# taaha-khan/2023-CompaCT-Image-Compression

Measured on AMD Instinct MI355X. Metric: MPixels/s encode+decode, 12-bit 512x512 CT batch, bytes-exact, higher is better.
Workload: dtype u16

## Files before the change

2023-compact-image-compression_amd/csrc/api.cpp:

```cpp
#include <dlfcn.h>
#include <unistd.h>
#include <zlib.h>

#include <atomic>
#include <chrono>
#include <condition_variable>
#include <functional>
#include <cstdarg>
#include <cstdio>
#include <cstdlib>
#include <cstring>
#include <map>
#include <mutex>
#include <string>
#include <thread>
#include <vector>

#include "../../include/compact_hip.h"
#include "cct_internal.h"
#include "host.h"
#include "handoff.h"

namespace cct {
bool gilbert_table(int width, int height, int32_t *out);
// ... 619 lines not shown
		return CCT_OK;
	}
	if (tb && tb->tiled) {
		bool tile_role_in_lds = true;
		(void)enc_tiles_lds_bytes(NB, &tile_role_in_lds);
		if (!tile_role_in_lds) { if ((rc = E.e_role.ensure(per))) return rc; a.ws_role = (uint8_t *)E.e_role.p; }
		else a.ws_role = nullptr;
		TileEncArgs ta{};
		ta.e = a;
		ta.tile_org = tb->d_org; ta.tile_orient = tb->d_orient; ta.patterns = tb->d_pat;
		ta.n_orient = tb->n_orient; ta.n_tiles = tb->n_tiles; ta.row_pitch = width;
		HIP_TRY(launch_encode_tiles(ta, n, st));
		g_ctx.last_path = 2;
		return CCT_OK;
	}
	const bool run_time = bs_run_time(bs, g_ctx.runtime_bs != 0);
	HIP_TRY(launch_encode(a, n, bs, g_ctx.wg_threads, st, run_time));
	g_ctx.last_path = run_time ? 4 : 0;
	return CCT_OK;
}

constexpr size_t DEFLATE_PASS_BYTES = (size_t)1 << 30;

int deflate_locked(EncSlot &E, const uint8_t *d_in, size_t in_stride, const uint32_t *d_in_sizes, int n, const uint8_t header13[13],
                   size_t out_stride, int level, int strategy, int mem_level = 8)
{
	if (in_stride % 256 != 0 || out_stride % 4 != 0) return fail(CCT_E_ARG, "deflate strides must be multiples of 256 / 4");
	DeflateArgs a{};
	if (!deflate_strategy_args(level, strategy, a))
		return fail(CCT_E_ARG, "zlib level %d with strategy %d is not on the device", level, strategy);
	if (!deflate_mem_level_args(mem_level, a)) return fail(CCT_E_ARG, "zlib memLevel %d: 8 and 9 are on the device", mem_level);
	const size_t EB = (size_t)n * in_stride;
	if (EB >= ((size_t)1 << 32)) return fail(CCT_E_ARG, "deflate batch of %zu bytes exceeds the 4 GiB sort limit; split the batch", EB);
	const DflShape shape = dfl_shape(n, in_stride, a.block_syms);
	int rc;
	void *base[DFL_REGIONS];
	for (int r = 0; r < DFL_REGIONS; r++) {
		if (dfl_region_needed(r, strategy) && (rc = E.z_ws[r].ensure(dfl_region_bytes(r, shape)))) return rc;
		base[r] = E.z_ws[r].p;
	}
	if ((rc = E.z_out.ensure((size_t)n * out_stride))) return rc;
	if ((rc = E.z_outsizes.ensure((size_t)n * 4))) return rc;
	const bool use_fork = g_ctx.deflate_fork != 0;
	if (use_fork && !E.stream_side) {
		const int crc = exclusive_section([&]() -> int { HIP_TRY(hipStreamCreateWithFlags(&E.stream_side, hipStreamNonBlocking)); return CCT_OK; });
		if (crc) return crc;
	}
	a.in = d_in; a.in_stride = in_stride; a.in_sizes = d_in_sizes;
	dfl_bind(a, base, shape);
	a.tree_waves = (uint32_t)g_ctx.tree_waves;
	a.pos_mask = (g_ctx.compact_recs && mem_level == 8 && in_stride < ((size_t)1 << 22)) ? (1u << 22) - 1u : 0xFFFFFFFFu;
	const DevBuf &mr = E.z_ws[DFL_R_MATCH];
	if (dfl_uses_chains(strategy)) {
		if (E.z_mr_cleared != mr.p || E.z_mr_cleared_cap != mr.cap || E.z_gen_passes >= 16000u) {
			HIP_TRY(hipMemsetAsync(mr.p, 0, mr.cap, E.stream));
			HIP_TRY(hipMemsetAsync(E.z_ws[DFL_R_GEN].p, 0, 256, E.stream));
			E.z_mr_cleared = mr.p; E.z_mr_cleared_cap = mr.cap; E.z_gen_passes = 0;
		}
		E.z_gen_passes++;
	}
	a.out = (uint8_t *)E.z_out.p; a.out_stride = out_stride; a.out_sizes = (uint32_t *)E.z_outsizes.p;
	memcpy(a.header13, header13, 13);
	if (g_ctx.use_graph) {
		std::vector<uint8_t> key(sizeof(DeflateArgs) + 2 * sizeof(int));
		memcpy(key.data(), &a, sizeof(DeflateArgs));
		memcpy(key.data() + sizeof(DeflateArgs), &n, sizeof(int));
		const int fork_key = use_fork ? 1 : 0;
		memcpy(key.data() + sizeof(DeflateArgs) + sizeof(int), &fork_key, sizeof(int));
		EncSlot::ZGraph *zg = nullptr;
		for (auto &g : E.z_graphs) if (g.key == key) zg = &g;
		if (!zg) {
			const int crc = exclusive_section([&]() -> int {
				if (E.z_graphs.size() >= 4) {
					size_t old = 0;
					for (size_t i = 1; i < E.z_graphs.size(); i++) if (E.z_graphs[i].last_use < E.z_graphs[old].last_use) old = i;
					if (E.z_graphs[old].exec) (void)hipGraphExecDestroy(E.z_graphs[old].exec);
					if (E.z_graphs[old].graph) (void)hipGraphDestroy(E.z_graphs[old].graph);
					E.z_graphs.erase(E.z_graphs.begin() + (long)old);
				}
				EncSlot::ZGraph g;
				HIP_TRY(hipStreamBeginCapture(E.stream, hipStreamCaptureModeThreadLocal));
				hipError_t le = launch_deflate(a, n, E.stream, use_fork ? E.stream_side : nullptr, E.ev_fork);
				hipError_t ce = hipStreamEndCapture(E.stream, &g.graph);
				if (le != hipSuccess) { if (g.graph) (void)hipGraphDestroy(g.graph); return fail(CCT_E_DEVICE, "DEFLATE capture: %s", hipGetErrorString(le)); }
				HIP_TRY(ce);
				const hipError_t ie = hipGraphInstantiate(&g.exec, g.graph, nullptr, nullptr, 0);
				if (ie != hipSuccess) { (void)hipGraphDestroy(g.graph); return fail(CCT_E_DEVICE, "hipGraphInstantiate failed: %s", hipGetErrorString(ie)); }
				g.key = key;
				E.z_graphs.push_back(std::move(g));
				return CCT_OK;
			});
			if (crc) return crc;
			zg = &E.z_graphs.back();
		}
		zg->last_use = ++E.z_clock;
		HIP_TRY(hipGraphLaunch(zg->exec, E.stream));
		return CCT_OK;
	}
	HIP_TRY(launch_deflate(a, n, E.stream, use_fork ? E.stream_side : nullptr, E.ev_fork));
	return CCT_OK;
}

int decode_payload_locked(DecSlot &D, const uint8_t *d_payload, size_t stride, const uint32_t *d_sizes, int n, int width,
                          int height, int bs, int fractal, uint16_t *d_images, uint32_t *d_status, hipStream_t st)
{
	const int N = width * height, NB = N / bs;
	if (stride % 16 != 0) return fail(CCT_E_ARG, "payload stride must be a multiple of 16");
// ... 1416 lines not shown
```

2023-compact-image-compression_amd/csrc/deflate_kernels.hip:

```cpp
#include <hip/hip_runtime.h>
#include <cstring>
#include <algorithm>

#include "cct_internal.h"
#include "wave_device.h"
#include "../../include/compact_hip.h"

namespace cct {
namespace {

constexpr int MIN_MATCH = 3, MAX_MATCH = 258, WSIZE = 32768;
constexpr int MIN_LOOKAHEAD = MAX_MATCH + MIN_MATCH + 1;
constexpr int MAX_DIST = WSIZE - MIN_LOOKAHEAD;
constexpr int TOO_FAR = 4096;
constexpr int BLOCK_SYMS = 16383;
constexpr int BLOCK_SYMS_ML9 = 32767;
constexpr int L_CODES = 286, D_CODES = 30, BL_CODES = 19, HEAP_SIZE = 2 * L_CODES + 1;
constexpr int END_BLOCK = 256, MAX_BITS = 15, MAX_BL_BITS = 7;
constexpr uint32_t Z_FILTERED = 1, Z_HUFFMAN_ONLY = 2, Z_RLE = 3, Z_FIXED = 4;
__host__ __device__ __forceinline__ bool short_pass(uint32_t strategy) { return strategy == Z_HUFFMAN_ONLY || strategy == Z_RLE; }

__constant__ uint8_t c_extra_lbits[29] = {0,0,0,0,0,0,0,0,1,1,1,1,2,2,2,2,3,3,3,3,4,4,4,4,5,5,5,5,0};
__constant__ uint8_t c_extra_dbits[30] = {0,0,0,0,1,1,2,2,3,3,4,4,5,5,6,6,7,7,8,8,9,9,10,10,11,11,12,12,13,13};
__constant__ uint8_t c_extra_blbits[19] = {0,0,0,0,0,0,0,0,0,0,0,0,0,0,0,0,2,3,7};
__constant__ uint8_t c_bl_order[19] = {16,17,18,0,8,7,9,6,10,5,11,4,12,3,13,2,14,1,15};
__constant__ uint8_t c_length_code[256];
__constant__ uint16_t c_base_length[29];
__constant__ uint8_t c_dist_code[512];
__constant__ uint16_t c_base_dist[30];
__constant__ uint16_t c_static_lcode[288];
__constant__ uint8_t c_static_llen[288];
__constant__ uint16_t c_static_dcode[30];

template <int HB>
__device__ __forceinline__ uint32_t hash3(uint32_t b0, uint32_t b1, uint32_t b2)
{
	constexpr int SH = (HB + 2) / 3;
	return ((b0 << (2 * SH)) ^ (b1 << SH) ^ b2) & ((1u << HB) - 1u);
}

__device__ __forceinline__ int d_code(uint32_t dist) { return dist < 256 ? c_dist_code[dist] : c_dist_code[256 + (dist >> 7)]; }

struct MatchRec { uint16_t len_full, len_quarter, dist_full, dist_quarter; };
constexpr uint32_t GEN_MAX = 16383;
__device__ __forceinline__ uint2 pack_match(uint32_t len_full, uint32_t len_quarter, uint32_t dist_full, uint32_t dist_quarter, uint32_t gen)
{
	return make_uint2((len_full | ((gen & 127u) << 9)) | ((len_quarter | ((gen >> 7) << 9)) << 16), dist_full | (dist_quarter << 16));
}
__device__ __forceinline__ MatchRec checked_match(MatchRec r, uint32_t gen, uint32_t rw, uint32_t p, uint32_t L)
{
	const uint32_t tag = (uint32_t)(r.len_full >> 9) | ((uint32_t)(r.len_quarter >> 9) << 7);
	const uint32_t lookahead = L - min(p, L);
	const uint32_t max_len = lookahead < (uint32_t)MAX_MATCH ? lookahead : (uint32_t)MAX_MATCH;
	const bool maximal = (rw >> 15) && (rw & 0x7FFFu) >= max_len && p + 2 < L;
	MatchRec o;
	const bool ok = tag == gen;
	o.len_full = ok ? (uint16_t)(r.len_full & 511u) : (uint16_t)(maximal ? max_len : 0u);
	o.len_quarter = ok ? (uint16_t)(r.len_quarter & 511u) : (uint16_t)(maximal ? max_len : 0u);
	o.dist_full = ok ? r.dist_full : (uint16_t)(maximal ? 1u : 0u);
	o.dist_quarter = ok ? r.dist_quarter : (uint16_t)(maximal ? 1u : 0u);
	return o;
}

template <bool FIRST, int HB>
__global__ void __launch_bounds__(1024) dfl_sort_pass_kernel(DeflateArgs a)
{
	constexpr int BITS = FIRST ? 8 : HB - 8, NB = 1 << BITS;
	constexpr uint32_t HMASK = (1u << HB) - 1u;
	__shared__ uint32_t offs[256];
	__shared__ uint32_t wcnt[16][NB];
	const int s = blockIdx.x;
	const uint32_t L = a.in_sizes[s];
	const uint8_t *in = a.in + (size_t)s * a.in_stride;
	const size_t base = (size_t)s * a.in_stride;
	const uint32_t npos = L >= MIN_MATCH ? L - 2 : 0;
	const uint64_t *rec_src = a.rec_in + base;
	uint64_t *rec_dst = (FIRST ? a.rec_in : a.rec_out) + base;
	const int tid = threadIdx.x, lane = tid & 63, wave = tid >> 6;
	const uint64_t lt_mask = (1ull << lane) - 1ull;
	if (tid < 256) offs[tid] = 0;
	__syncthreads();
	if (tid < NB) offs[tid] = a.sort_hist[(size_t)s * SORT_HIST + (FIRST ? 0 : 256) + tid];
	__syncthreads();
	if (wave == 0) {
		uint32_t v[4], sum = 0;
#pragma unroll
		for (int k = 0; k < 4; k++) { v[k] = offs[lane * 4 + k]; sum += v[k]; }
		uint32_t run = wave_incl_scan(sum) - sum;
#pragma unroll
		for (int k = 0; k < 4; k++) { offs[lane * 4 + k] = run; run += v[k]; }
	}
	__syncthreads();
#ifndef CCT_SORT_E
#define CCT_SORT_E 4
#endif
	constexpr int E = CCT_SORT_E;
	constexpr int ND = E / 4;
	const uint32_t last = npos ? npos - 1 : 0;
	static_assert(E % 4 == 0 && ND + 1 <= E, "pass A: whole dwords per lane, kept in ra[0 .. ND]");
#ifdef CCT_SORT_PROBE
	const bool compact = false;
#else
	const bool compact = HB == 15 && a.pos_mask != 0xFFFFFFFFu;
#endif
	const uint32_t dmax = (uint32_t)a.in_stride - 4u;
	auto fetch = [&](uint32_t tile_base, uint32_t (&ra)[E], uint32_t (&rb)[E]) {
		if (FIRST) {
#pragma unroll
			for (int d = 0; d < ND; d++) ra[d] = *reinterpret_cast<const uint32_t *>(in + min(tile_base + 256u * d + 4u * (uint32_t)lane, dmax));
			ra[ND] = *reinterpret_cast<const uint32_t *>(in + min(tile_base + 256u * ND, dmax));
#pragma unroll
			for (int e = 0; e < E; e++) rb[e] = compact ? a.run_len[base + min(tile_base + (uint32_t)(e * 64 + lane), last)] : 0u;
		} else {
// ... 259 lines not shown
		if ((rw >> 15) && (int)run_r >= nice_eff) { best = best1 = (int)run_r; best_q = best_q1 = p - 1; }
		else kind = 2;
		return;
	}
	for (int64_t j = (int64_t)i - 1; j >= 0; j--) {
		const uint64_t rj = recs[j];
		if (rec_hash(rj, pos_mask) != h) break;
		if (count == LIGHT_STEPS) { kind = 1; break; }
		const uint32_t q = rec_pos(rj, pos_mask);
		const uint32_t dist = p - q;
		if (q == 0 || q == nil_q) break;
		if (count == 0 ? dist > (uint32_t)MAX_DIST : dist >= (uint32_t)MAX_DIST) break;
		const uint8_t *mp = in + q;
		{
			int len = 0;
			if (wide) {
				if (best < 8 || mp[best] == sp[best]) {
					uint64_t cw;
					__builtin_memcpy(&cw, mp, 8);
					const uint64_t d = cw ^ ow;
					len = d ? (__ffsll((long long)d) - 1) >> 3 : common_prefix(mp, sp, 8, max_len);
				}
			} else if (mp[best] == sp[best]) len = common_prefix(mp, sp, 0, max_len);
			if (len > best) {
				best = len; best_q = q;
				if (count < quarter) { best1 = len; best_q1 = q; }
			}
		}
		count++;
		if (best >= nice_eff) break;
	}
}

#ifndef DFL_MATCH_Q
#define DFL_MATCH_Q 256
#endif
#ifndef DFL_MATCH_GRID
#define DFL_MATCH_GRID 32
#endif
constexpr uint32_t MATCH_Q = DFL_MATCH_Q;
static_assert(MATCH_Q >= 128 && (MATCH_Q & 63) == 0, "a turn appends up to 64 entries to a list");

template <bool CMP, bool QL>
__global__ void __launch_bounds__(256) dfl_match_kernel(DeflateArgs a, int n)
{
	__shared__ uint32_t queue[4][2][MATCH_Q];
	int s; uint32_t part, nparts;
	if (!xcd_slice(n, s, part, nparts)) return;
	const uint32_t L = a.in_sizes[s], gen = *a.gen;
	const uint8_t *in = a.in + (size_t)s * a.in_stride;
	const size_t base = (size_t)s * a.in_stride;
	const uint32_t npos = L >= MIN_MATCH ? L - 2 : 0;
	const uint64_t *recs = a.rec_out + base;
	uint2 *mr = reinterpret_cast<uint2 *>(a.mr) + base;
	uint32_t *heavy = a.heavy_list + base;
	const uint16_t *rl = a.run_len + base;
	const int lane = threadIdx.x & 63;
	const uint64_t lt_mask = (1ull << lane) - 1ull;
	const int quarter = QL ? (int)(a.max_chain >> 2) : LIGHT_STEPS + 1;
	const uint32_t stride = nparts * 256u;
	uint32_t i0 = part * 256u;
	if (i0 >= npos) return;
	uint32_t *qh = queue[threadIdx.x >> 6][0], *qr = queue[threadIdx.x >> 6][1];
	uint32_t nh = 0, nr = 0;
	auto flush = [&](const uint32_t *q, uint32_t cnt, uint32_t *counter, bool down) {
		uint32_t b = 0;
		if (lane == 0) b = atomicAdd(counter, cnt);
		b = (uint32_t)__builtin_amdgcn_readfirstlane((int)b);
		__builtin_amdgcn_wave_barrier();
		for (uint32_t k = (uint32_t)lane; k < cnt; k += 64u) {
			if (down) *(dfl_deep_top(heavy, a.in_stride) - (b + k)) = q[k];
			else heavy[b + k] = q[k];
		}
		__builtin_amdgcn_wave_barrier();
	};
	auto rec_at = [&](uint32_t i) { return recs[min(i, npos - 1)]; };
	auto rec_before = [&](uint32_t i) { return recs[min(i >= 64 ? i - 64 : 0u, npos - 1)]; };
	uint64_t ri_next = rec_at(i0 + threadIdx.x), rb_next = CMP ? rec_before(i0 + threadIdx.x) : 0ull;
	for (; i0 < npos; i0 += stride) {
		const uint32_t i = i0 + threadIdx.x;
		const bool valid = i < npos;
		int kind = 0;
		int best = 0, best1 = 0;
		uint32_t best_q = 0, best_q1 = 0, run_r = 0;
		const uint64_t ri = ri_next, rb = rb_next;
		ri_next = rec_at(i + stride);
		if (CMP) rb_next = rec_before(i + stride);
		const uint32_t p = rec_pos(ri, CMP ? COMPACT_POS_MASK : 0xFFFFFFFFu);
		const uint32_t h = rec_hash(ri, CMP ? COMPACT_POS_MASK : 0xFFFFFFFFu);
		bool from_memory = valid;
		bool found = false;
		if (CMP) {
			const uint32_t lo_i = (uint32_t)ri, hi_i = (uint32_t)(ri >> 32), lo_b = (uint32_t)rb, hi_b = (uint32_t)(rb >> 32);
			const uint32_t lookahead = L - p;
			const int max_len = lookahead < (uint32_t)MAX_MATCH ? (int)lookahead : MAX_MATCH;
			const int nice_eff = (int)min(lookahead, a.nice);
			const bool fast = valid && p + 8 <= L;
			from_memory = valid && !fast;
			const uint32_t nil_q = nil_candidate(p, lookahead);
			const uint32_t b1 = (lo_i >> 22) & 255u;
			const bool in_run = h == (((b1 << 10) ^ (b1 << 5) ^ b1) & 0x7FFFu) && (((lo_i >> 30) | ((hi_i >> 31) << 2)) == (b1 >> 5));
			if (fast && in_run) {
				const uint32_t rw = (hi_i >> 15) & 0xFFFFu;
				run_r = rw & 0x7FFFu;
				if (!((rw >> 15) && (int)run_r >= nice_eff)) kind = 2;
				else if ((int)run_r < max_len) { best = best1 = (int)run_r; best_q = best_q1 = p - 1; found = true; }
			}
			bool act = fast && !in_run;
			const uint32_t qmin_head = (p > (uint32_t)MAX_DIST ? p - (uint32_t)MAX_DIST : 1u) + (nil_q != 0xFFFFFFFFu ? 1u : 0u);
			const uint32_t qmin_rest = p >= (uint32_t)MAX_DIST ? p - (uint32_t)MAX_DIST + 1u : 1u;
			const uint32_t steps_i = min(i, (uint32_t)LIGHT_STEPS + 1u);
			uint32_t clo = lo_i, chi = hi_i;
#pragma unroll
			for (int k = 1; k <= LIGHT_STEPS + 1; k++) {
				clo = wave_shift_up(clo, (uint32_t)__builtin_amdgcn_readlane((int)lo_b, 64 - k));
				chi = wave_shift_up(chi, (uint32_t)__builtin_amdgcn_readlane((int)hi_b, 64 - k));
				if (!__any(act)) break;
				const uint32_t x = hi_i ^ chi;
				const uint32_t q = clo & COMPACT_POS_MASK;
				if ((uint32_t)k > steps_i || (x & 0x7FFFu) != 0 || q < (k == 1 ? qmin_head : qmin_rest)) act = false;
				if (act) {
					if (k == LIGHT_STEPS + 1) { kind = 1; act = false; }
					else {
						if (best < nice_eff && (((lo_i ^ clo) >> 22) | (x >> 31)) == 0) {
							int len;
							if (x & 0x007F8000u) len = 3;
							else if (x) len = 4;
							else if (best < 5 || in[q + best] == in[p + best]) len = common_prefix(in + q, in + p, 5, max_len);
							else len = 0;
							if (len > best) {
								best = len; best_q = q; found = true;
								if (QL && k <= quarter) { best1 = len; best_q1 = q; }
							}
						}
						if (best >= nice_eff) act = false;
					}
				}
			}
		}
		if (from_memory) {
			light_match_from_memory(in, recs, rl, CMP ? COMPACT_POS_MASK : 0xFFFFFFFFu, L, i, p, h, a.nice, quarter, kind, best, best_q,
			                        best1, best_q1, run_r);
			found = kind == 0 && best >= MIN_MATCH;
		}
		if (found && kind == 0) {
			if (!QL) { best1 = best; best_q1 = best_q; }
			mr[p] = pack_match((uint32_t)best, (uint32_t)best1, p - best_q, best1 ? p - best_q1 : 0u, gen);
		}
		const uint64_t bh = __ballot(kind == 1), br = __ballot(kind == 2);
		if (kind == 1) qh[nh + (uint32_t)__popcll(bh & lt_mask)] = i;
		if (kind == 2) qr[nr + (uint32_t)__popcll(br & lt_mask)] = i;
		nh += (uint32_t)__popcll(bh); nr += (uint32_t)__popcll(br);
		if (nh > MATCH_Q - 64u) { flush(qh, nh, &a.heavy_count[s], false); nh = 0; }
		if (nr > MATCH_Q - 64u) { flush(qr, nr, &a.deep_count[s], true); nr = 0; }
	}
	if (nh) flush(qh, nh, &a.heavy_count[s], false);
	if (nr) flush(qr, nr, &a.deep_count[s], true);
}

__device__ __forceinline__ void coop_longest_match(const uint8_t *in, const uint64_t *recs, uint32_t L,
                                                   uint32_t i, uint32_t p, uint32_t pos_mask, int lane, uint32_t nice, uint32_t max_chain,
                                                   uint32_t &lo, uint32_t &hi)
{
	const uint32_t h = rec_hash(recs[i], pos_mask);
	const uint32_t lookahead = L - p;
	const int max_len = lookahead < (uint32_t)MAX_MATCH ? (int)lookahead : MAX_MATCH;
	const int nice_eff = (int)min(lookahead, nice);
	const uint32_t quarter = max_chain >> 2;
	const int steps = (int)((max_chain + 63) >> 6);
	const uint32_t nil_q = nil_candidate(p, lookahead);
	const uint8_t *sp = in + p;
	int best = 0;
	uint32_t best_q = 0;
	int len_q = -1;
	uint32_t q_q = 0;
	auto pick = [&](uint64_t cand, int len, uint32_t q, int &b_len, uint32_t &b_q) {
		for (int b = 8; b >= 0; b--) {
			const uint64_t mb = __ballot((len >> b) & 1) & cand;
			if (mb) cand = mb;
		}
		const int win = __builtin_amdgcn_readfirstlane(__ffsll((long long)cand) - 1);
		b_len = __builtin_amdgcn_readlane(len, win);
		b_q = (uint32_t)__builtin_amdgcn_readlane((int)q, win);
	};
	auto rec_of_round = [&](int r) { const int64_t j = (int64_t)i - 1 - (int64_t)(r * 64 + lane); return recs[j >= 0 ? j : 0]; };
	uint64_t rj_next = rec_of_round(0);
	for (int r = 0; r < steps; r++) {
		const int64_t j = (int64_t)i - 1 - (int64_t)(r * 64 + lane);
		const uint64_t rj = j >= 0 ? rj_next : ~0ull;
		rj_next = rec_of_round(r + 1);
		const bool in_chain = j >= 0 && rec_hash(rj, pos_mask) == h && (uint32_t)(r * 64 + lane) < max_chain;
		const uint32_t q = in_chain ? rec_pos(rj, pos_mask) : 0u;
		const uint32_t dist = p - q;
		const bool term = !in_chain || q == 0 || q == nil_q ||
		                  ((r == 0 && lane == 0) ? dist > (uint32_t)MAX_DIST : dist >= (uint32_t)MAX_DIST);
		const uint64_t tmask = __ballot(term);
		const int nvalid = tmask ? (__ffsll((long long)tmask) - 1) : 64;
		int len = 0;
		if (lane < nvalid) {
			const uint8_t *mp = in + q;
			if (mp[best] == sp[best]) len = common_prefix(mp, sp, 0, max_len);
		}
		const uint64_t nice_m = __ballot(len >= nice_eff);
		const uint64_t upto = nice_m ? ((nice_m & (0 - nice_m)) << 1) - 1u : ~0ull;
		const int best_before = best;
		const uint32_t best_q_before = best_q;
		const uint64_t cand = __ballot(len > best_before) & upto;
		if (cand) pick(cand, len, q, best, best_q);
		const uint32_t qb = quarter - (uint32_t)(r * 64);
		if ((uint32_t)(r * 64) < quarter && qb <= 64u) {
			const uint64_t cq = cand & (qb == 64u ? ~0ull : (1ull << qb) - 1u);
			if (cq == cand) { len_q = best; q_q = best_q; }
			else if (cq) pick(cq, len, q, len_q, q_q);
			else { len_q = best_before; q_q = best_q_before; }
		}
		if (nice_m || nvalid < 64) break;
	}
	if (len_q < 0) { len_q = best; q_q = best_q; }
	lo = (uint32_t)best | ((uint32_t)len_q << 16);
	hi = (best ? p - best_q : 0u) | ((len_q ? p - q_q : 0u) << 16);
}

__global__ void __launch_bounds__(256) dfl_match_heavy_kernel(DeflateArgs a, int n)
{
	int s; uint32_t part, nparts;
	if (!xcd_slice(n, s, part, nparts)) return;
	const uint32_t L = a.in_sizes[s];
	const uint8_t *in = a.in + (size_t)s * a.in_stride;
	const size_t base = (size_t)s * a.in_stride;
	const uint64_t *recs = a.rec_out + base;
	uint2 *mr = reinterpret_cast<uint2 *>(a.mr) + base;
	const uint32_t *heavy = a.heavy_list + base;
	const uint32_t nheavy = a.heavy_count[s];
	const int lane = threadIdx.x & 63;
	const uint32_t gen = *a.gen;
	for (uint32_t e = part * (blockDim.x >> 6) + (threadIdx.x >> 6); e < nheavy; e += nparts * (blockDim.x >> 6)) {
		const uint32_t i = heavy[e];
		const uint32_t p = rec_pos(recs[i], a.pos_mask);
		uint32_t lo, hi;
		coop_longest_match(in, recs, L, i, p, a.pos_mask, lane, a.nice, a.max_chain, lo, hi);
		if (lane == 0) mr[p] = pack_match(lo & 0xFFFFu, lo >> 16, hi & 0xFFFFu, hi >> 16, gen);
	}
}

__global__ void __launch_bounds__(256) dfl_run_lists_kernel(DeflateArgs a)
{
	__shared__ uint32_t wsum[4], base_es[2];
	const int s = blockIdx.y;
	const uint32_t L = a.in_sizes[s];
	const uint32_t c = blockIdx.x;
	const uint32_t c0 = c * RUNLEN_OUT;
	if (c0 >= L) return;
	const uint8_t *in = a.in + (size_t)s * a.in_stride;
	const uint16_t *rl = a.run_len + (size_t)s * a.in_stride;
	uint32_t *re = a.run_ends + (size_t)s * a.in_stride;
	uint32_t *rs = dfl_run_starts(re, a.in_stride);
	const uint32_t *cnt = a.run_counts + (size_t)s * 2 * a.run_chunks;
	const int tid = threadIdx.x, lane = tid & 63, wave = tid >> 6;
	const uint32_t g = c0 + (uint32_t)tid * 8;
	uint4 wv = make_uint4(0, 0, 0, 0);
	if (tid * 8 < RUNLEN_OUT && g < L) wv = *reinterpret_cast<const uint4 *>(rl + g);
	const bool first_two_equal = L >= 2 && in[0] == in[1];
	if (wave == 0) {
		uint32_t be = 0, bs = 0;
		for (uint32_t q = lane; q < c; q += 64) { be += cnt[2 * q]; bs += cnt[2 * q + 1]; }
		be = wave_sum(be); bs = wave_sum(bs);
		if (lane == 0) { base_es[0] = be; base_es[1] = bs; }
	}
	const uint32_t w32[4] = {wv.x, wv.y, wv.z, wv.w};
	uint32_t me = 0, ms = 0;
#pragma unroll
	for (int k = 0; k < 8; k++) {
		const uint32_t w = (w32[k >> 1] >> (16 * (k & 1))) & 0xFFFFu, r = w & 0x7FFFu, p = g + (uint32_t)k;
		const bool pub = (uint32_t)tid * 8 + k < (uint32_t)RUNLEN_OUT && p < L;
		const bool prev_eq = p >= 2 ? (w >> 15) != 0 : (p == 1 && first_two_equal);
		me |= (uint32_t)(pub && r == 3u && p + 3 < L) << k;
		ms |= (uint32_t)(pub && r >= 3u && !prev_eq) << k;
	}
	uint32_t tot;
	const uint32_t ex = wg_excl_scan<4>((uint32_t)__popc(me) | (uint32_t)__popc(ms) << 16, wsum, tot);
	uint32_t ie = base_es[0] + (ex & 0xFFFFu), is = base_es[1] + (ex >> 16);
	const uint32_t tot_e = base_es[0] + (tot & 0xFFFFu);
	if ((uint32_t)tid * 8 < (uint32_t)RUNLEN_OUT && g < L) re[dfl_run_rank(a.in_stride, g)] = ie;
#pragma unroll
	for (int k = 0; k < 8; k++) {
		if ((me >> k) & 1u) re[ie++] = g + k + 3;
		if ((ms >> k) & 1u) rs[is++] = g + k;
	}
	if (tid == 0 && c0 + RUNLEN_OUT >= L) a.run_end_count[s] = tot_e;
}

__global__ void __launch_bounds__(256) dfl_run_info_kernel(DeflateArgs a)
{
	const int s = blockIdx.y;
	const uint8_t *in = a.in + (size_t)s * a.in_stride;
	const uint32_t *re = a.run_ends + (size_t)s * a.in_stride;
	const uint32_t *rs = dfl_run_starts(re, a.in_stride);
	uint32_t *rl = dfl_run_info(a.run_ends + (size_t)s * a.in_stride, a.in_stride);
	const uint32_t nre = a.run_end_count[s];
	for (uint32_t t = blockIdx.x * blockDim.x + threadIdx.x; t < nre; t += gridDim.x * blockDim.x) {
		const uint32_t x = re[t], len = x - rs[t];
		rl[t] = (len < 511u ? len : 511u) | ((uint32_t)in[x - 1] << 16);
	}
}

__global__ void __launch_bounds__(256) dfl_match_run_kernel(DeflateArgs a, int n)
{
	int s; uint32_t part, nparts;
	if (!xcd_slice(n, s, part, nparts)) return;
	const uint32_t L = a.in_sizes[s];
	const uint8_t *in = a.in + (size_t)s * a.in_stride;
	const size_t base = (size_t)s * a.in_stride;
	const uint64_t *recs = a.rec_out + base;
	uint2 *mr = reinterpret_cast<uint2 *>(a.mr) + base;
	const uint32_t *deep = dfl_deep_top(a.heavy_list + base, a.in_stride);
	const uint32_t ndeep = a.deep_count[s];
	const uint32_t *re = a.run_ends + base;
	const uint32_t *rl = dfl_run_info(re, a.in_stride);
	const uint32_t nre = a.run_end_count[s];
	const uint32_t gen = *a.gen;
	const uint32_t quarter = a.max_chain >> 2;
	for (uint32_t e = part * blockDim.x + threadIdx.x; e < ndeep; e += nparts * blockDim.x) {
		const uint32_t i = *(deep - e);
		const uint64_t ri = recs[i];
		const uint64_t r_head = recs[i >= 1 ? i - 1 : 0], r_quarter = recs[i >= quarter ? i - quarter : 0], r_full = recs[i >= a.max_chain ? i - a.max_chain : 0];
		const uint32_t p = rec_pos(ri, a.pos_mask);
		const uint32_t h = rec_hash(ri, a.pos_mask);
		const uint32_t lookahead = L - p;
		const uint32_t max_len = lookahead < (uint32_t)MAX_MATCH ? lookahead : (uint32_t)MAX_MATCH;
		const uint32_t nice_eff = min(lookahead, a.nice);
		const uint8_t b = in[p], b_prev = in[p >= 1 ? p - 1 : 0];
		const uint32_t r = a.run_len[base + p] & 0x7FFFu;
		const uint32_t k = min(r, nice_eff);
		const bool has_prev = p >= 2 && b_prev == b;
		uint32_t best4 = has_prev ? r : 0u, q4 = p - 1, best1 = best4, q1 = p - 1;
		bool scan = true;
		if (!has_prev) {
			const uint64_t rh = i >= 1 ? r_head : ~0ull;
			const bool have_head = i >= 1 && rec_hash(rh, a.pos_mask) == h;
			const uint32_t hq = have_head ? rec_pos(rh, a.pos_mask) : 0u;
			if (!have_head || hq == 0 || hq == nil_candidate(p, lookahead) || p - hq > (uint32_t)MAX_DIST) scan = false;
			else if (p - hq == (uint32_t)MAX_DIST) {
				uint32_t len = 0;
				len = (uint32_t)common_prefix(in + hq, in + p, 0, (int)max_len);
				best4 = best1 = len; q4 = q1 = hq;
				scan = false;
			}
		}
		if (scan && best4 < nice_eff) {
			const bool ext_ok = r < max_len;
			const uint8_t c = ext_ok ? in[p + r] : 0;
			const uint32_t qw = p >= (uint32_t)MAX_DIST ? p - (uint32_t)MAX_DIST + 1 : 1u;
			uint32_t qmin4 = qw, qmin1 = qw;
			if (i >= a.max_chain && rec_hash(r_full, a.pos_mask) == h) qmin4 = max(qmin4, rec_pos(r_full, a.pos_mask));
			if (i >= quarter && rec_hash(r_quarter, a.pos_mask) == h) qmin1 = max(qmin1, rec_pos(r_quarter, a.pos_mask));
			uint32_t lo = 0;
			if (p >= 3) {
				lo = re[dfl_run_rank(a.in_stride, p - 2)];
				while (lo < nre && re[lo] <= p) lo++;
			}
			uint32_t x_n = lo ? re[lo - 1] : 0u, lw_n = lo ? rl[lo - 1] : 0u;
			for (int64_t t = (int64_t)lo - 1; t >= 0; t--) {
				const uint32_t x = x_n;
				const uint32_t lw = lw_n;
				{ const int64_t tn = t > 0 ? t - 1 : 0; x_n = re[tn]; lw_n = rl[tn]; }
				if (x < qmin4 + 3) break;
				if ((lw >> 16) != b) continue;
				const uint32_t m = min(min(lw & 0xFFFFu, k), x - qmin4);
				if (m >= 3) {
					uint32_t q, len;
					if (m == r) {
						q = x - r; len = r;
						if (ext_ok && in[x] == c) len = (uint32_t)common_prefix(in + q, in + p, (int)r + 1, (int)max_len);
					} else { q = x - m; len = m; }
					if (len > best4) { best4 = len; q4 = q; }
					if (x >= qmin1 + 3) {
						const uint32_t m1 = min(m, x - qmin1);
						if (m1 == m) { if (len > best1) { best1 = len; q1 = q; } }
						else if (m1 >= 3 && m1 > best1) { best1 = m1; q1 = x - m1; }
					}
					if (best4 >= nice_eff) break;
				}
				if (x - m <= qmin4) break;
			}
		}
		mr[p] = pack_match(best4, best1, best4 ? p - q4 : 0u, best1 ? p - q1 : 0u, gen);
	}
}

__device__ __forceinline__ void match_of(const MatchRec &r, uint32_t p, uint32_t npos, int prev_len, int lazy, int good, int minl,
                                         int &len, int &dist)
{
	len = 2; dist = 0;
	if (p >= npos || prev_len >= lazy) return;
	const int l = prev_len >= good ? r.len_quarter : r.len_full;
	const int d = prev_len >= good ? r.dist_quarter : r.dist_full;
	if (l > prev_len && l >= minl) { len = l; dist = d; }
	if (len == MIN_MATCH && dist > TOO_FAR) len = 2;
}
__device__ __forceinline__ void match_at(const MatchRec *mr, const uint16_t *rl, uint32_t gen, uint32_t p, uint32_t npos, int prev_len,
                                         int lazy, int good, int minl, int &len, int &dist)
{
	len = 2; dist = 0;
	if (p >= npos || prev_len >= lazy) return;
	match_of(checked_match(mr[p], gen, rl[p], p, npos + 2), p, npos, prev_len, lazy, good, minl, len, dist);
}

__global__ void __launch_bounds__(256) dfl_rec_kernel(DeflateArgs a)
{
	const int s = blockIdx.y;
	const uint32_t L = a.in_sizes[s];
	const size_t base = (size_t)s * a.in_stride;
	const uint32_t npos = L >= MIN_MATCH ? L - 2 : 0;
	const MatchRec *mr = reinterpret_cast<const MatchRec *>(a.mr) + base;
	const uint16_t *rl = a.run_len + base;
	const uint32_t nblk64 = (L + 63) / 64;
	const int lane = threadIdx.x & 63;
	const uint32_t gen = *a.gen;
	const int lazy = (int)a.max_lazy, good = (int)a.good, minl = (int)a.min_len;
	const uint32_t lastp = npos ? npos - 1 : 0;
	const uint32_t wb_step = gridDim.x * (blockDim.x >> 6);
	struct Req { MatchRec m0, m1; uint32_t w0, w1; };
	auto request = [&](uint32_t wb) {
		const uint32_t p = wb * 64 + lane, pa = min(p, lastp), pb = min(p + 1, lastp);
		return Req{mr[pa], mr[pb], rl[pa], rl[pb]};
	};
	const uint32_t wb0 = blockIdx.x * (blockDim.x >> 6) + (threadIdx.x >> 6);
	Req nx = request(wb0);
	for (uint32_t wb = wb0; wb < nblk64; wb += wb_step) {
		const uint32_t p = wb * 64 + lane;
		const uint32_t blk_end = wb * 64 + 64;
		uint32_t rec = 0, nxt = blk_end, cnt = 0;
		const uint32_t pa = min(p, lastp), pb = min(p + 1, lastp);
		const Req cq = nx;
		nx = request(wb + wb_step);
		const MatchRec r0 = checked_match(cq.m0, gen, cq.w0, pa, L), r1 = checked_match(cq.m1, gen, cq.w1, pb, L);
		if (p < L) {
			int len, dist;
			match_of(r0, p, npos, 2, lazy, good, minl, len, dist);
			if (len < MIN_MATCH) { rec = 0; nxt = p + 1; cnt = 1; }
			else {
				uint32_t k = 0;
				for (;;) {
					int l2, d2;
					if (k == 0) match_of(r1, p + 1, npos, len, lazy, good, minl, l2, d2);
					else match_at(mr, rl, gen, p + k + 1, npos, len, lazy, good, minl, l2, d2);
					if (l2 > len) { len = l2; dist = d2; k++; } else break;
				}
				rec = k | ((uint32_t)len << 8) | ((uint32_t)dist << 17);
				nxt = p + k + (uint32_t)len;
				cnt = k + 1;
			}
		}
		a.rec32[base + p] = rec;
#pragma unroll
		for (int r = 0; r < 6; r++) {
			const bool inside = nxt < blk_end;
			const int j = inside ? (int)(nxt - wb * 64) : lane;
			const uint32_t n2 = __shfl(nxt, j), c2 = __shfl(cnt, j);
			if (inside) { nxt = n2; cnt += c2; }
		}
		a.exit_pos[base + p] = (nxt - blk_end) | (cnt << 16);
	}
}

__global__ void __launch_bounds__(256) dfl_rle_rec_kernel(DeflateArgs a)
{
	const int s = blockIdx.y;
	const uint32_t L = a.in_sizes[s];
	const size_t base = (size_t)s * a.in_stride;
	const uint16_t *rl = a.run_len + base;
	const uint32_t nblk64 = (L + 63) / 64;
	const int lane = threadIdx.x & 63;
	const uint32_t lastp = L ? L - 1 : 0;
	const uint32_t wb_step = gridDim.x * (blockDim.x >> 6);
	const uint32_t wb0 = blockIdx.x * (blockDim.x >> 6) + (threadIdx.x >> 6);
	uint32_t nx = rl[min(wb0 * 64 + lane, lastp)];
	for (uint32_t wb = wb0; wb < nblk64; wb += wb_step) {
		const uint32_t p = wb * 64 + lane;
		const uint32_t blk_end = wb * 64 + 64;
		const uint32_t rw = nx;
		nx = rl[min((wb + wb_step) * 64 + lane, lastp)];
		const uint32_t rw0 = (uint32_t)__shfl((int)rw, 0);
		const bool prev_eq = p >= 2 ? (rw >> 15) != 0 : (p == 1 && (rw0 & 0x7FFFu) >= 2u);
		const uint32_t run = rw & 0x7FFFu;
		uint32_t rec = 0, nxt = blk_end, cnt = 0;
		if (p < L) {
			const bool m = prev_eq && run >= (uint32_t)MIN_MATCH;
			rec = m ? (run << 8) | (1u << 17) : 0u;
			nxt = p + (m ? run : 1u);
			cnt = 1;
		}
		a.rec32[base + p] = rec;
#pragma unroll
		for (int r = 0; r < 6; r++) {
			const bool inside = nxt < blk_end;
			const int j = inside ? (int)(nxt - wb * 64) : lane;
			const uint32_t n2 = __shfl(nxt, j), c2 = __shfl(cnt, j);
			if (inside) { nxt = n2; cnt += c2; }
// ... 944 lines not shown
		const uint32_t nwords = ((uint32_t)(run & 31) + tot + 31) >> 5;
		const uint64_t gw = run >> 5;
		for (uint32_t k = threadIdx.x; k < nwords; k += blockDim.x) {
			const uint32_t w = wbf[k];
			wbf[k] = 0;
			if (k == 0 || k == nwords - 1) { if (w) atomicOr(&words[gw + k], w); }
			else words[gw + k] = w;
		}
		run += tot;
	}
}

__global__ void __launch_bounds__(256) dfl_pack_offsets_kernel(const uint32_t *sizes, int n, uint64_t *offsets, int exact)
{
	__shared__ uint64_t wsum[4];
	const int t = threadIdx.x, lane = t & 63, wave = t >> 6;
	uint64_t carry = 0;
	for (int base = 0; base < n; base += 256) {
		const int i = base + t;
		const uint32_t sz = i < n ? sizes[i] : 0u;
		const uint64_t v = exact ? sz : (uint64_t)((sz + 15u) & ~15u);
		const uint64_t inc = wave_incl_scan(v);
		if (lane == 63) wsum[wave] = inc;
		__syncthreads();
		uint64_t wb = 0, tot = 0;
		for (int w = 0; w < 4; w++) { if (w < wave) wb += wsum[w]; tot += wsum[w]; }
		if (i < n) offsets[i] = carry + wb + inc - v;
		carry += tot;
		__syncthreads();
	}
	if (t == 0) offsets[n] = carry;
}
__global__ void __launch_bounds__(256) dfl_pack_kernel(const uint8_t *src, size_t stride, const uint32_t *sizes,
                                                       const uint64_t *offsets, uint8_t *dst)
{
	const int s = blockIdx.y;
	const uint32_t n16 = (sizes[s] + 15u) >> 4;
	const uint4 *in = reinterpret_cast<const uint4 *>(src + (size_t)s * stride);
	uint4 *out = reinterpret_cast<uint4 *>(dst + offsets[s]);
	for (uint32_t i = blockIdx.x * blockDim.x + threadIdx.x; i < n16; i += gridDim.x * blockDim.x) out[i] = in[i];
}

__global__ void dfl_offsets2_kernel(DeflateArgs a, int n)
{
	const size_t per = dfl_blk_words(a.in_stride);
	for (size_t i = blockIdx.x * (size_t)blockDim.x + threadIdx.x; i < (size_t)n * per; i += (size_t)gridDim.x * blockDim.x)
		a.blk_entry[i] = 0xFFFFFFFFu;
}

__global__ void dfl_offsets_kernel(DeflateArgs a, int n)
{
	if (blockIdx.x == 0) {
		for (int s = threadIdx.x; s < n; s += blockDim.x) { a.postloop_lit[s] = 0; a.heavy_count[s] = 0; a.deep_count[s] = 0; a.run_end_count[s] = 0; }
		if (threadIdx.x == 0) *a.gen = *a.gen % GEN_MAX + 1u;
	}
	const size_t nrc = dfl_hist_words((size_t)n, (size_t)a.run_chunks);
	for (size_t t = (size_t)blockIdx.x * blockDim.x + threadIdx.x; t < nrc; t += (size_t)gridDim.x * blockDim.x) a.sort_hist[t] = 0;
}

constexpr uint32_t CLEAR_SLACK = 64;
__device__ __forceinline__ size_t clear_bytes(const DeflateArgs &a, int s)
{
	const size_t L = a.in_sizes[s];
	const size_t bound = a.block_syms == (uint32_t)BLOCK_SYMS ? L + (L >> 12) + (L >> 14) + (L >> 25) + 13
	                                                          : L + ((L + 7) >> 3) + ((L + 63) >> 6) + 5 + 6;
	return min(a.out_stride, (13 + bound + CLEAR_SLACK + 15) & ~(size_t)15);
}
template <typename W>
__global__ void __launch_bounds__(256) dfl_clear_kernel(DeflateArgs a)
{
	const int s = blockIdx.y;
	const size_t units = clear_bytes(a, s) / sizeof(W);
	W *out = reinterpret_cast<W *>(a.out + (size_t)s * a.out_stride);
	W zero{};
	for (size_t i = blockIdx.x * (size_t)blockDim.x + threadIdx.x; i < units; i += (size_t)gridDim.x * blockDim.x) out[i] = zero;
}
static void launch_clear(const DeflateArgs &a, int n, hipStream_t st)
{
	if (a.out_stride % 16 == 0 && (uintptr_t)a.out % 16 == 0) hipLaunchKernelGGL(dfl_clear_kernel<uint4>, dim3(16, n), dim3(256), 0, st, a);
	else hipLaunchKernelGGL(dfl_clear_kernel<uint32_t>, dim3(32, n), dim3(256), 0, st, a);
}

}

bool deflate_level_args(int level, DeflateArgs &a)
{
	static const uint32_t T[6][5] = {
		{4, 4, 16, 16, 0x5E}, {8, 16, 32, 32, 0x5E}, {8, 16, 128, 128, 0x9C},
		{8, 32, 128, 256, 0xDA}, {32, 128, 258, 1024, 0xDA}, {32, 258, 258, 4096, 0xDA},
	};
	if (level < 4 || level > 9) return false;
	const uint32_t *t = T[level - 4];
	a.good = t[0]; a.max_lazy = t[1]; a.nice = t[2]; a.max_chain = t[3]; a.zlib_flg = t[4];
	return true;
}

bool deflate_strategy_args(int level, int strategy, DeflateArgs &a)
{
	if (strategy < 0 || strategy > (int)Z_FIXED) return false;
	a.strategy = (uint32_t)strategy;
	a.min_len = strategy == (int)Z_FILTERED ? 6u : (uint32_t)MIN_MATCH;
	if (short_pass((uint32_t)strategy)) {
		if (level < 1 || level > 9) return false;
		a.good = a.max_lazy = a.nice = a.max_chain = 0;
		a.zlib_flg = 0x01;
		return true;
	}
// ... 198 lines not shown
```

2023-compact-image-compression_amd/csrc/deflate_workspace.h:

```cpp
#pragma once
#include <stddef.h>
#include <stdint.h>

#if defined(__HIPCC__)
#include <hip/hip_runtime.h>
#define DFL_HD __host__ __device__ __forceinline__
#else
#define DFL_HD inline
#endif

namespace cct {

struct BlockMeta {
	uint64_t bit_off;
	uint32_t type;
	uint32_t last;
	uint32_t first_sym, nsym;
	uint32_t in_begin, stored_len;
	uint32_t hdr_nbits, body_bits;
};
struct BlockTables {
	uint16_t lcode[286]; uint8_t llen[286];
	uint16_t dcode[30]; uint8_t dlen[30];
	uint32_t hdr_bits[160];
};
struct DeflateArgs {
	const uint8_t *in; size_t in_stride; const uint32_t *in_sizes;
	uint64_t *rec_in, *rec_out;
	uint32_t pos_mask;
	uint32_t *seg_begin, *seg_end;
	void *mr;
	uint32_t *gen;
	uint32_t *heavy_list, *sym, *run_ends;
	uint32_t *run_counts; int run_chunks;
	uint32_t *sort_hist;
	uint16_t *run_len;
	uint32_t *rec32, *exit_pos, *exit_cnt;
	uint32_t *blk_entry, *blk_symbase;
	uint32_t *total_syms, *postloop_lit, *n_blocks, *adler, *heavy_count, *deep_count, *run_end_count;
	uint32_t *blk_end;
	uint32_t *blk_top;
	BlockMeta *block_meta; BlockTables *block_tables;
	int max_blocks;
	uint8_t *out; size_t out_stride; uint32_t *out_sizes;
	uint8_t header13[16];
	uint32_t good, max_lazy, nice, max_chain, zlib_flg;
	uint32_t strategy, min_len;
	uint32_t hash_bits, block_syms;
	uint32_t tree_waves;
};

constexpr int SORT_HIST = 512;
constexpr int RUNLEN_OUT = 2048 - 264;
constexpr int BLK_ENTRY_GRAIN = 64;
enum DflCounter { DFL_SEG_BEGIN, DFL_SEG_END, DFL_TOTAL_SYMS, DFL_POSTLOOP_LIT, DFL_N_BLOCKS, DFL_ADLER, DFL_HEAVY_COUNT,
// ... 37 lines not shown
inline bool dfl_region_needed(int r, int strategy)
{
	return DFL_REGION_NEED[r] == DFL_ALWAYS || (DFL_REGION_NEED[r] == DFL_CHAINS ? dfl_uses_chains(strategy) : strategy != 2);
}

struct DflShape { size_t n, in_stride, max_blocks, run_chunks; };
inline DflShape dfl_shape(int n, size_t in_stride, uint32_t block_syms)
{
	return {(size_t)n, in_stride, (size_t)dfl_max_blocks(in_stride, block_syms), (size_t)dfl_run_chunks(in_stride)};
}
inline size_t dfl_region_bytes(int r, const DflShape &w)
{
	const size_t EB = w.n * w.in_stride;
	switch (r) {
	case DFL_R_REC_IN: case DFL_R_REC_OUT: case DFL_R_MATCH: return EB * 8;
	case DFL_R_RUNS: case DFL_R_QUEUES: case DFL_R_SYM: case DFL_R_REC32: case DFL_R_EXIT_POS: return EB * 4;
	case DFL_R_BLK_ENTRY: case DFL_R_BLK_SYMBASE: return EB / BLK_ENTRY_GRAIN * 4;
	case DFL_R_SMALL: return (DFL_COUNTERS * w.n + dfl_hist_words(w.n, w.run_chunks)) * 4;
	case DFL_R_BLK_ENDS: return w.n * w.max_blocks * 8;
	case DFL_R_META: return w.n * w.max_blocks * sizeof(BlockMeta);
	case DFL_R_TABLES: return w.n * w.max_blocks * sizeof(BlockTables);
	case DFL_R_GEN: return 256;
	}
	return 0;
}

inline void dfl_bind(DeflateArgs &a, void *const base[DFL_REGIONS], const DflShape &w)
{
	a.rec_in = (uint64_t *)base[DFL_R_REC_IN]; a.rec_out = (uint64_t *)base[DFL_R_REC_OUT];
	a.mr = base[DFL_R_MATCH]; a.gen = (uint32_t *)base[DFL_R_GEN];
	a.run_ends = (uint32_t *)base[DFL_R_RUNS];
	a.heavy_list = (uint32_t *)base[DFL_R_QUEUES];
	a.exit_cnt = (uint32_t *)base[DFL_R_QUEUES];
	a.sym = (uint32_t *)base[DFL_R_SYM];
	a.run_len = (uint16_t *)base[DFL_R_SYM];
	a.rec32 = (uint32_t *)base[DFL_R_REC32]; a.exit_pos = (uint32_t *)base[DFL_R_EXIT_POS];
	a.blk_entry = (uint32_t *)base[DFL_R_BLK_ENTRY]; a.blk_symbase = (uint32_t *)base[DFL_R_BLK_SYMBASE];
	uint32_t *small = (uint32_t *)base[DFL_R_SMALL];
	a.seg_begin = small + DFL_SEG_BEGIN * w.n; a.seg_end = small + DFL_SEG_END * w.n; a.total_syms = small + DFL_TOTAL_SYMS * w.n;
	a.postloop_lit = small + DFL_POSTLOOP_LIT * w.n; a.n_blocks = small + DFL_N_BLOCKS * w.n; a.adler = small + DFL_ADLER * w.n;
	a.heavy_count = small + DFL_HEAVY_COUNT * w.n; a.deep_count = small + DFL_DEEP_COUNT * w.n;
	a.run_end_count = small + DFL_RUN_END_COUNT * w.n;
	a.sort_hist = small + DFL_COUNTERS * w.n;
	a.run_counts = a.sort_hist + SORT_HIST * w.n;
	a.run_chunks = (int)w.run_chunks;
	a.blk_end = (uint32_t *)base[DFL_R_BLK_ENDS]; a.blk_top = a.blk_end + w.n * w.max_blocks;
	a.block_meta = (BlockMeta *)base[DFL_R_META]; a.block_tables = (BlockTables *)base[DFL_R_TABLES];
	a.max_blocks = (int)w.max_blocks;
}

template <class T> DFL_HD T *dfl_run_starts(T *re, size_t in_stride) { return re + (in_stride >> 2); }
template <class T> DFL_HD T *dfl_run_info(T *re, size_t in_stride) { return re + (in_stride >> 1); }
DFL_HD size_t dfl_run_rank(size_t in_stride, uint32_t p) { return 3 * (in_stride >> 2) + (p >> 3); }
template <class T> DFL_HD T *dfl_deep_top(T *q, size_t in_stride) { return q + in_stride - 1; }

}
```

Before: 18350.

## Split match records into 32-bit primary word plus sparse quarter word

Replaces the 8-byte per-position match record with a 32-bit primary word holding the full-chain length, distance, a same-bit and a 7-bit generation tag. The quarter-chain result moves to a separate array that is written and read only when it differs from the full result. The aim is to halve the memory traffic of match writes and of the reads in the lazy-evaluation record kernel. In exchange the tag shrinks from 14 to 7 bits, so the full match buffer is cleared far more often (every ~100 passes instead of every 16000).

```diff
diff --git a/2023-compact-image-compression_amd/csrc/api.cpp b/2023-compact-image-compression_amd/csrc/api.cpp
--- a/2023-compact-image-compression_amd/csrc/api.cpp
+++ b/2023-compact-image-compression_amd/csrc/api.cpp
@@ -695,7 +695,7 @@
 	a.pos_mask = (g_ctx.compact_recs && mem_level == 8 && in_stride < ((size_t)1 << 22)) ? (1u << 22) - 1u : 0xFFFFFFFFu;
 	const DevBuf &mr = E.z_ws[DFL_R_MATCH];
 	if (dfl_uses_chains(strategy)) {
-		if (E.z_mr_cleared != mr.p || E.z_mr_cleared_cap != mr.cap || E.z_gen_passes >= 16000u) {
+		if (E.z_mr_cleared != mr.p || E.z_mr_cleared_cap != mr.cap || E.z_gen_passes >= MATCH_TAG_CLEAR_AFTER) {
 			HIP_TRY(hipMemsetAsync(mr.p, 0, mr.cap, E.stream));
 			HIP_TRY(hipMemsetAsync(E.z_ws[DFL_R_GEN].p, 0, 256, E.stream));
 			E.z_mr_cleared = mr.p; E.z_mr_cleared_cap = mr.cap; E.z_gen_passes = 0;
diff --git a/2023-compact-image-compression_amd/csrc/deflate_kernels.hip b/2023-compact-image-compression_amd/csrc/deflate_kernels.hip
--- a/2023-compact-image-compression_amd/csrc/deflate_kernels.hip
+++ b/2023-compact-image-compression_amd/csrc/deflate_kernels.hip
@@ -41,24 +41,24 @@
 
 __device__ __forceinline__ int d_code(uint32_t dist) { return dist < 256 ? c_dist_code[dist] : c_dist_code[256 + (dist >> 7)]; }
 
-struct MatchRec { uint16_t len_full, len_quarter, dist_full, dist_quarter; };
-constexpr uint32_t GEN_MAX = 16383;
-__device__ __forceinline__ uint2 pack_match(uint32_t len_full, uint32_t len_quarter, uint32_t dist_full, uint32_t dist_quarter, uint32_t gen)
-{
-	return make_uint2((len_full | ((gen & 127u) << 9)) | ((len_quarter | ((gen >> 7) << 9)) << 16), dist_full | (dist_quarter << 16));
-}
-__device__ __forceinline__ MatchRec checked_match(MatchRec r, uint32_t gen, uint32_t rw, uint32_t p, uint32_t L)
-{
-	const uint32_t tag = (uint32_t)(r.len_full >> 9) | ((uint32_t)(r.len_quarter >> 9) << 7);
+__device__ __forceinline__ void store_match(uint32_t *mr, uint32_t *mq, uint32_t p, uint32_t len_full, uint32_t len_quarter,
+                                            uint32_t dist_full, uint32_t dist_quarter, uint32_t gen)
+{
+	const MatchWords w = match_pack(len_full, dist_full, len_quarter, dist_quarter, gen);
+	mr[p] = w.primary;
+	if (w.has_secondary) mq[p] = w.secondary;
+}
+struct MatchRec { uint32_t len_full, dist_full; bool split; };
+__device__ __forceinline__ MatchRec checked_match(uint32_t primary, uint32_t gen, uint32_t rw, uint32_t p, uint32_t L)
+{
+	const MatchFull m = match_unpack(primary, gen);
 	const uint32_t lookahead = L - min(p, L);
 	const uint32_t max_len = lookahead < (uint32_t)MAX_MATCH ? lookahead : (uint32_t)MAX_MATCH;
 	const bool maximal = (rw >> 15) && (rw & 0x7FFFu) >= max_len && p + 2 < L;
 	MatchRec o;
-	const bool ok = tag == gen;
-	o.len_full = ok ? (uint16_t)(r.len_full & 511u) : (uint16_t)(maximal ? max_len : 0u);
-	o.len_quarter = ok ? (uint16_t)(r.len_quarter & 511u) : (uint16_t)(maximal ? max_len : 0u);
-	o.dist_full = ok ? r.dist_full : (uint16_t)(maximal ? 1u : 0u);
-	o.dist_quarter = ok ? r.dist_quarter : (uint16_t)(maximal ? 1u : 0u);
+	o.len_full = m.valid ? m.len : (maximal ? max_len : 0u);
+	o.dist_full = m.valid ? m.dist : (maximal ? 1u : 0u);
+	o.split = m.valid && !m.same;
 	return o;
 }
 
@@ -424,7 +424,8 @@
 	const size_t base = (size_t)s * a.in_stride;
 	const uint32_t npos = L >= MIN_MATCH ? L - 2 : 0;
 	const uint64_t *recs = a.rec_out + base;
-	uint2 *mr = reinterpret_cast<uint2 *>(a.mr) + base;
+	uint32_t *mr = reinterpret_cast<uint32_t *>(a.mr) + base;
+	uint32_t *mq = dfl_match_quarter(mr, (size_t)n, a.in_stride);
 	uint32_t *heavy = a.heavy_list + base;
 	const uint16_t *rl = a.run_len + base;
 	const int lane = threadIdx.x & 63;
@@ -517,7 +518,7 @@
 		}
 		if (found && kind == 0) {
 			if (!QL) { best1 = best; best_q1 = best_q; }
-			mr[p] = pack_match((uint32_t)best, (uint32_t)best1, p - best_q, best1 ? p - best_q1 : 0u, gen);
+			store_match(mr, mq, p, (uint32_t)best, (uint32_t)best1, p - best_q, best1 ? p - best_q1 : 0u, gen);
 		}
 		const uint64_t bh = __ballot(kind == 1), br = __ballot(kind == 2);
 		if (kind == 1) qh[nh + (uint32_t)__popcll(bh & lt_mask)] = i;
@@ -601,7 +602,8 @@
 	const uint8_t *in = a.in + (size_t)s * a.in_stride;
 	const size_t base = (size_t)s * a.in_stride;
 	const uint64_t *recs = a.rec_out + base;
-	uint2 *mr = reinterpret_cast<uint2 *>(a.mr) + base;
+	uint32_t *mr = reinterpret_cast<uint32_t *>(a.mr) + base;
+	uint32_t *mq = dfl_match_quarter(mr, (size_t)n, a.in_stride);
 	const uint32_t *heavy = a.heavy_list + base;
 	const uint32_t nheavy = a.heavy_count[s];
 	const int lane = threadIdx.x & 63;
@@ -611,7 +613,7 @@
 		const uint32_t p = rec_pos(recs[i], a.pos_mask);
 		uint32_t lo, hi;
 		coop_longest_match(in, recs, L, i, p, a.pos_mask, lane, a.nice, a.max_chain, lo, hi);
-		if (lane == 0) mr[p] = pack_match(lo & 0xFFFFu, lo >> 16, hi & 0xFFFFu, hi >> 16, gen);
+		if (lane == 0) store_match(mr, mq, p, lo & 0xFFFFu, lo >> 16, hi & 0xFFFFu, hi >> 16, gen);
 	}
 }
 
@@ -684,7 +686,8 @@
 	const uint8_t *in = a.in + (size_t)s * a.in_stride;
 	const size_t base = (size_t)s * a.in_stride;
 	const uint64_t *recs = a.rec_out + base;
-	uint2 *mr = reinterpret_cast<uint2 *>(a.mr) + base;
+	uint32_t *mr = reinterpret_cast<uint32_t *>(a.mr) + base;
+	uint32_t *mq = dfl_match_quarter(mr, (size_t)n, a.in_stride);
 	const uint32_t *deep = dfl_deep_top(a.heavy_list + base, a.in_stride);
 	const uint32_t ndeep = a.deep_count[s];
 	const uint32_t *re = a.run_ends + base;
@@ -756,26 +759,29 @@
 				if (x - m <= qmin4) break;
 			}
 		}
-		mr[p] = pack_match(best4, best1, best4 ? p - q4 : 0u, best1 ? p - q1 : 0u, gen);
-	}
-}
-
-__device__ __forceinline__ void match_of(const MatchRec &r, uint32_t p, uint32_t npos, int prev_len, int lazy, int good, int minl,
-                                         int &len, int &dist)
+		store_match(mr, mq, p, best4, best1, best4 ? p - q4 : 0u, best1 ? p - q1 : 0u, gen);
+	}
+}
+
+__device__ __forceinline__ void match_of(const MatchRec &r, const uint32_t *mq, uint32_t p, uint32_t npos, int prev_len, int lazy, int good,
+                                         int minl, int &len, int &dist)
 {
 	len = 2; dist = 0;
 	if (p >= npos || prev_len >= lazy) return;
-	const int l = prev_len >= good ? r.len_quarter : r.len_full;
-	const int d = prev_len >= good ? r.dist_quarter : r.dist_full;
+	int l = (int)r.len_full, d = (int)r.dist_full;
+	if (prev_len >= good && r.split) {
+		const MatchQuarter q = match_unpack_secondary(mq[p]);
+		l = (int)q.len; d = (int)q.dist;
+	}
 	if (l > prev_len && l >= minl) { len = l; dist = d; }
 	if (len == MIN_MATCH && dist > TOO_FAR) len = 2;
 }
-__device__ __forceinline__ void match_at(const MatchRec *mr, const uint16_t *rl, uint32_t gen, uint32_t p, uint32_t npos, int prev_len,
-                                         int lazy, int good, int minl, int &len, int &dist)
+__device__ __forceinline__ void match_at(const uint32_t *mr, const uint32_t *mq, const uint16_t *rl, uint32_t gen, uint32_t p, uint32_t npos,
+                                         int prev_len, int lazy, int good, int minl, int &len, int &dist)
 {
 	len = 2; dist = 0;
 	if (p >= npos || prev_len >= lazy) return;
-	match_of(checked_match(mr[p], gen, rl[p], p, npos + 2), p, npos, prev_len, lazy, good, minl, len, dist);
+	match_of(checked_match(mr[p], gen, rl[p], p, npos + 2), mq, p, npos, prev_len, lazy, good, minl, len, dist);
 }
 
 __global__ void __launch_bounds__(256) dfl_rec_kernel(DeflateArgs a)
@@ -784,7 +790,8 @@
 	const uint32_t L = a.in_sizes[s];
 	const size_t base = (size_t)s * a.in_stride;
 	const uint32_t npos = L >= MIN_MATCH ? L - 2 : 0;
-	const MatchRec *mr = reinterpret_cast<const MatchRec *>(a.mr) + base;
+	const uint32_t *mr = reinterpret_cast<const uint32_t *>(a.mr) + base;
+	const uint32_t *mq = dfl_match_quarter(mr, (size_t)gridDim.y, a.in_stride);
 	const uint16_t *rl = a.run_len + base;
 	const uint32_t nblk64 = (L + 63) / 64;
 	const int lane = threadIdx.x & 63;
@@ -792,7 +799,7 @@
 	const int lazy = (int)a.max_lazy, good = (int)a.good, minl = (int)a.min_len;
 	const uint32_t lastp = npos ? npos - 1 : 0;
 	const uint32_t wb_step = gridDim.x * (blockDim.x >> 6);
-	struct Req { MatchRec m0, m1; uint32_t w0, w1; };
+	struct Req { uint32_t m0, m1, w0, w1; };
 	auto request = [&](uint32_t wb) {
 		const uint32_t p = wb * 64 + lane, pa = min(p, lastp), pb = min(p + 1, lastp);
 		return Req{mr[pa], mr[pb], rl[pa], rl[pb]};
@@ -809,14 +816,14 @@
 		const MatchRec r0 = checked_match(cq.m0, gen, cq.w0, pa, L), r1 = checked_match(cq.m1, gen, cq.w1, pb, L);
 		if (p < L) {
 			int len, dist;
-			match_of(r0, p, npos, 2, lazy, good, minl, len, dist);
+			match_of(r0, mq, p, npos, 2, lazy, good, minl, len, dist);
 			if (len < MIN_MATCH) { rec = 0; nxt = p + 1; cnt = 1; }
 			else {
 				uint32_t k = 0;
 				for (;;) {
 					int l2, d2;
-					if (k == 0) match_of(r1, p + 1, npos, len, lazy, good, minl, l2, d2);
-					else match_at(mr, rl, gen, p + k + 1, npos, len, lazy, good, minl, l2, d2);
+					if (k == 0) match_of(r1, mq, p + 1, npos, len, lazy, good, minl, l2, d2);
+					else match_at(mr, mq, rl, gen, p + k + 1, npos, len, lazy, good, minl, l2, d2);
 					if (l2 > len) { len = l2; dist = d2; k++; } else break;
 				}
 				rec = k | ((uint32_t)len << 8) | ((uint32_t)dist << 17);
@@ -1867,7 +1874,7 @@
 {
 	if (blockIdx.x == 0) {
 		for (int s = threadIdx.x; s < n; s += blockDim.x) { a.postloop_lit[s] = 0; a.heavy_count[s] = 0; a.deep_count[s] = 0; a.run_end_count[s] = 0; }
-		if (threadIdx.x == 0) *a.gen = *a.gen % GEN_MAX + 1u;
+		if (threadIdx.x == 0) *a.gen = match_next_tag(*a.gen);
 	}
 	const size_t nrc = dfl_hist_words((size_t)n, (size_t)a.run_chunks);
 	for (size_t t = (size_t)blockIdx.x * blockDim.x + threadIdx.x; t < nrc; t += (size_t)gridDim.x * blockDim.x) a.sort_hist[t] = 0;
diff --git a/2023-compact-image-compression_amd/csrc/deflate_match_record.h b/2023-compact-image-compression_amd/csrc/deflate_match_record.h
--- /dev/null
+++ b/2023-compact-image-compression_amd/csrc/deflate_match_record.h
@@ -0,0 +1,54 @@
+#pragma once
+#include <stdint.h>
+
+#if defined(__HIPCC__)
+#include <hip/hip_runtime.h>
+#define MREC_HD __host__ __device__ __forceinline__
+#else
+#define MREC_HD inline
+#endif
+
+namespace cct {
+
+constexpr uint32_t MATCH_LEN_BITS = 9, MATCH_DIST_BITS = 15, MATCH_TAG_BITS = 7;
+constexpr uint32_t MATCH_LEN_MASK = (1u << MATCH_LEN_BITS) - 1u, MATCH_DIST_MASK = (1u << MATCH_DIST_BITS) - 1u;
+constexpr uint32_t MATCH_SAME_BIT = 1u << (MATCH_LEN_BITS + MATCH_DIST_BITS);
+constexpr uint32_t MATCH_TAG_SHIFT = MATCH_LEN_BITS + MATCH_DIST_BITS + 1;
+static_assert(MATCH_TAG_SHIFT + MATCH_TAG_BITS == 32, "a primary word is 32 bits");
+constexpr uint32_t MATCH_TAG_MAX = (1u << MATCH_TAG_BITS) - 1u;
+constexpr uint32_t MATCH_TAG_CLEAR_AFTER = MATCH_TAG_MAX - 27u;
+
+struct MatchWords { uint32_t primary, secondary; bool has_secondary; };
+struct MatchFull { uint32_t len, dist; bool valid, same; };
+struct MatchQuarter { uint32_t len, dist; };
+
+MREC_HD uint32_t match_next_tag(uint32_t tag) { return tag % MATCH_TAG_MAX + 1u; }
+
+MREC_HD uint32_t match_pack_secondary(uint32_t len_quarter, uint32_t dist_quarter) { return len_quarter | (dist_quarter << MATCH_LEN_BITS); }
+MREC_HD MatchWords match_pack(uint32_t len_full, uint32_t dist_full, uint32_t len_quarter, uint32_t dist_quarter, uint32_t tag)
+{
+	const bool same = len_full == len_quarter && dist_full == dist_quarter;
+	MatchWords w;
+	w.primary = len_full | (dist_full << MATCH_LEN_BITS) | (same ? MATCH_SAME_BIT : 0u) | (tag << MATCH_TAG_SHIFT);
+	w.secondary = match_pack_secondary(len_quarter, dist_quarter);
+	w.has_secondary = !same;
+	return w;
+}
+MREC_HD MatchFull match_unpack(uint32_t primary, uint32_t tag)
+{
+	MatchFull m;
+	m.valid = (primary >> MATCH_TAG_SHIFT) == tag;
+	m.len = primary & MATCH_LEN_MASK;
+	m.dist = (primary >> MATCH_LEN_BITS) & MATCH_DIST_MASK;
+	m.same = (primary & MATCH_SAME_BIT) != 0;
+	return m;
+}
+MREC_HD MatchQuarter match_unpack_secondary(uint32_t secondary)
+{
+	MatchQuarter q;
+	q.len = secondary & MATCH_LEN_MASK;
+	q.dist = (secondary >> MATCH_LEN_BITS) & MATCH_DIST_MASK;
+	return q;
+}
+
+}
diff --git a/2023-compact-image-compression_amd/csrc/deflate_workspace.h b/2023-compact-image-compression_amd/csrc/deflate_workspace.h
--- a/2023-compact-image-compression_amd/csrc/deflate_workspace.h
+++ b/2023-compact-image-compression_amd/csrc/deflate_workspace.h
@@ -1,6 +1,8 @@
 #pragma once
 #include <stddef.h>
 #include <stdint.h>
+
+#include "deflate_match_record.h"
 
 #if defined(__HIPCC__)
 #include <hip/hip_runtime.h>
@@ -144,6 +146,7 @@
 template <class T> DFL_HD T *dfl_run_starts(T *re, size_t in_stride) { return re + (in_stride >> 2); }
 template <class T> DFL_HD T *dfl_run_info(T *re, size_t in_stride) { return re + (in_stride >> 1); }
 DFL_HD size_t dfl_run_rank(size_t in_stride, uint32_t p) { return 3 * (in_stride >> 2) + (p >> 3); }
+template <class T> DFL_HD T *dfl_match_quarter(T *primary, size_t n, size_t in_stride) { return primary + n * in_stride; }
 template <class T> DFL_HD T *dfl_deep_top(T *q, size_t in_stride) { return q + in_stride - 1; }
 
 }
```

Result: no change. 18410 (median of 2 runs) (+0.3%).
